# Yubo-Shankui/Bind-Your-Avatar-Implementation

Hardware: AMD Instinct MI355X
Metric: denoise-steps/sec (higher is better)
Workload: dtype bf16; 1 GPU; BASELINE.json configs[1]: full transformer.forward, 49x480x720 (13x30x45 latent tokens + 226 text), 2 characters (2 ID + 2 audio), batch 1, random-init 8.6B-param architecture; layers=42, batch=1, launch=eager, parallelism=single GPU

## Files before the change

### bind_your_avatar_implementation_amd/_hip.py

```python
import ctypes
import os

from .build import LIB_PATH as _BUILT_LIB

LIB_PATH = os.environ.get("BYA_HIP_LIB") or _BUILT_LIB

_c = ctypes
_vp, _i32, _i64, _f32 = _c.c_void_p, _c.c_int32, _c.c_int64, _c.c_float


class GemmDesc(_c.Structure):
    _fields_ = [("M", _i32), ("N", _i32), ("K", _i32), ("batch", _i32),
                ("lda", _i32), ("ldw", _i32), ("ldc", _i32), ("ldres", _i32),
                ("a_batch_stride", _i64), ("c_batch_stride", _i64), ("res_batch_stride", _i64),
                ("gate_batch_stride", _i64), ("gate_split", _i32), ("act", _i32),
                ("n_split", _i32), ("c_split_stride", _i64), ("bias_rowscale", _vp), ("alpha", _f32)]


class GemmPlan(_c.Structure):
    _fields_ = [("path", _i32), ("m0", _i32), ("tail", _i32), ("split_k", _i32), ("row_chunks", _i32)]


class QkNormDesc(_c.Structure):
    _fields_ = [("qw", _vp), ("qb", _vp), ("kw", _vp), ("kb", _vp), ("cos", _vp), ("sin", _vp),
# ... 165 lines not shown
                                 _i32, _i64, _i32, _vp],
    "bya_vae_conv3d": [_vp, _vp, _vp, _vp, _vp, _i32, _i32, _i32, _i32, _i32, _i32, _i64, _i64, _i64, _vp],
    "bya_vae_upsample_pad": [_vp, _vp, _i32, _i32, _i32, _i32, _i32, _vp],
    "bya_allgather_kv": [_vp, _vp, _vp, _vp, _i64, _i64, _vp, _vp],
    "bya_alltoall_router": [_vp, _vp, _vp, _vp, _i32, _vp, _vp],
    "bya_p2p_push": [_vp, _i32, _i64, _vp, _i32, _i32, _vp, _vp],
    "bya_p2p_wait": [_vp, _i32, _vp, _i64, _vp],
    "bya_p2p_exchange": [_vp, _i32, _i64, _vp, _i32, _i32, _vp, _vp, _i64, _vp],
    "bya_p2p_push_verified": [_vp, _i32, _i64, _vp, _i32, _i32, _vp, _vp, _vp, _vp, _vp, _vp],
    "bya_p2p_exchange_verified": [_vp, _i32, _i64, _vp, _i32, _i32, _vp, _vp, _i64, _vp, _vp, _vp, _vp, _vp],
    "bya_p2p_verify": [_vp, _vp, _vp, _i32, _i32, _vp, _vp, _vp],
    "bya_p2p_poison": [_vp, _i32, _vp, _i64, _vp],
    "bya_p2p_alloc": [_i64, _i32, _c.POINTER(_vp)],
    "bya_p2p_free": [_vp],
    "bya_p2p_ipc_export": [_vp, _vp],
    "bya_p2p_ipc_import": [_vp, _c.POINTER(_vp)],
    "bya_p2p_ipc_release": [_vp],
    "bya_cfg_scheduler_step": [_vp, _i32, _i64, _vp, _vp, _vp, _vp, _vp, _i64, _c.POINTER(SchedCoef), _vp],
    "bya_cfg_scheduler_step_plan": [_vp, _i32, _i64, _vp, _vp, _i64, _c.POINTER(SchedCoef), _c.POINTER(StepPlan)],
}

OPTIONS = {"gemm_splitk": 0, "gemm_splitk_min": 1, "gemm_tile": 2, "gemm_variant": 3, "attn_streamk": 4, "fp8_kernel": 5,
           "p2p_groups": 6, "reference_forms": 7, "mx_kernel": 8}
REFERENCE_FORMS = {"rowgemm_chunked": 1, "kv_mix_generic": 2, "ln_generic": 4, "router_scores_wave": 8, "attn_narrow_store": 16}
def _named_value(var, v, table):
    if v not in table:
        raise ValueError(f"{var}={v!r}: expected one of {sorted(table)}")
    return table[v]


ENV_OPTIONS = {
    "BYA_GEMM_SPLITK": ("gemm_splitk", int),
    "BYA_GEMM_SPLITK_MIN": ("gemm_splitk_min", int),
    "BYA_GEMM_TILE": ("gemm_tile", int),
    "BYA_GEMM_VARIANT": ("gemm_variant", lambda v: {"w8": 1, "no128": 2}.get(v, 0)),
    "BYA_ATTN_STREAMK": ("attn_streamk", int),
    "BYA_FP8_KERNEL": ("fp8_kernel", lambda v: 1 if v.startswith("1") else 0),
    "BYA_P2P_GROUPS": ("p2p_groups", int),
    "BYA_MX_KERNEL": ("mx_kernel", lambda v: _named_value("BYA_MX_KERNEL", v, {"0": 0, "1": 1, "p256": 1, "2": 2, "always": 2})),
}

GEMM_PATHS = {0: "t128x64", 1: "t128x128", 2: "t256x128", 3: "t256x256", 4: "p256", 5: "p128", 6: "p128s", 7: "w8_256"}

ATTN_VARIANTS = {0: "d64_running_max", 1: "d64_prescaled_running_max", 2: "d64_static_bound", 3: "d128_running_max",
                 4: "d64_static_bound_w4", 5: "d64_device_bound_w4"}
KV_MIX_FORMS = {0: "mix32", 1: "one_tile"}
TINY_INSTANCES = {0: "tiny8<2>", 1: "tiny8<3>", 2: "tiny8<13>", 3: "tiny8<25>", 4: "generic<2>", 5: "generic<4>",
# ... 61 lines not shown
```

### bind_your_avatar_implementation_amd/csrc/gemm_persistent.h

```cpp
#pragma once
#include "gemm_common.h"

namespace {

typedef int i32x4 __attribute__((ext_vector_type(4)));

struct XcdRange { int base, end; };
__host__ __device__ __forceinline__ XcdRange xcd_range(int total, int xcd) {
    const int cq = total >> 3, cr = total & 7;
    const int base = (xcd < cr) ? xcd * (cq + 1) : cr * (cq + 1) + (xcd - cr) * cq;
    return {base, base + cq + (xcd < cr ? 1 : 0)};
}

struct PersistentTile { int z, m0, n0; bool valid; };

template <int BM, int BN>
struct TileWalk {
    int tiles_m, tiles_n, per_z, gm;
    int base, end, slot, slots;
    __device__ __forceinline__ TileWalk(int tiles_m_, int tiles_n_, int batch, int gm_)
        : tiles_m(tiles_m_), tiles_n(tiles_n_), per_z(tiles_m_ * tiles_n_), gm(gm_) {
        const int total = per_z * batch, xcd = blockIdx.x & 7;
        slot = blockIdx.x >> 3;
        slots = gridDim.x >> 3;
// ... 34 lines not shown
__device__ __forceinline__ uint32_t stage_off96(int lane, int q, int rl, int src_row, uint32_t pitch) {
    const int b = (q * 1024 + lane * 16) % 96;
    return (uint32_t)src_row * pitch + (uint32_t)((b + 48 * ((rl >> 3) & 1)) % 96);
}

__device__ __forceinline__ i32x4 raw_rsrc(const void* base, uint32_t bytes) {
    const unsigned long long b = (unsigned long long)base;
    i32x4 r;
    r.x = __builtin_amdgcn_readfirstlane((int)(b & 0xffffffffu));
    r.y = __builtin_amdgcn_readfirstlane((int)((b >> 32) & 0xffffu));
    r.z = __builtin_amdgcn_readfirstlane((int)bytes);
    r.w = 0x00020000;
    return r;
}

template <int LDS_OFF = 0>
__device__ __forceinline__ void dma_piece(uint32_t lds_base, uint32_t voff, const i32x4& rsrc, uint32_t soff) {
    asm volatile("s_mov_b32 m0, %0\n\ts_nop 0\n\tbuffer_load_dwordx4 %1, %2, %3 offen lds"
                 :
                 : "s"(lds_base + LDS_OFF), "v"(voff), "s"(rsrc), "s"(soff)
                 : "memory");
}

template <typename T>
__device__ __forceinline__ i32x4 tile_rsrc_a(const GemmArgs& p, const T* A, const PersistentTile& c, int row_elems = 0) {
    const long long left = ((long long)(p.M - 1 - c.m0) * p.lda + (row_elems ? row_elems : p.K)) * (long long)sizeof(T);
    return raw_rsrc(A + (long long)c.z * p.a_bs + (long long)c.m0 * p.lda, c.valid && left > 0 ? (uint32_t)left : 0u);
}
template <typename T>
__device__ __forceinline__ i32x4 tile_rsrc_w(const GemmArgs& p, const T* W, const PersistentTile& c, int row_elems = 0) {
    const long long left = ((long long)(p.N - 1 - c.n0) * p.ldw + (row_elems ? row_elems : p.K)) * (long long)sizeof(T);
    return raw_rsrc(W + (long long)c.n0 * p.ldw, c.valid && left > 0 ? (uint32_t)left : 0u);
}

__device__ __forceinline__ uint32_t frag_addr(uint32_t tile, int row, int chunk) {
    return tile + row * 128 + ((chunk ^ ((row >> 1) & 7)) << 4);
}

__device__ __forceinline__ uint32_t frag_addr64(uint32_t tile, int row, int chunk) {
    return tile + row * 64 + ((chunk ^ (((row >> 2) & 1) << 1)) << 4);
}

__device__ __forceinline__ uint32_t frag_addr96(uint32_t tile, int row, int blk) {
    return tile + row * 96 + (blk ^ (((row >> 3) & 1) << 1)) * 24;
}

// ... 19 lines not shown
```

### bind_your_avatar_implementation_amd/csrc/gemm_v4.hip

```cpp
#include "gemm_wide_epilogue.h"
#include "options.h"

#ifndef BYA_GEMM_ABLATE
#define BYA_GEMM_ABLATE 0
#endif

namespace {

#ifdef BYA_GEMM_TIMELINE
#define TL_STAMP(K) do { if (!SPLIT && tid == 0 && p.ws_slabs) tl[K] = __builtin_amdgcn_s_memrealtime(); } while (0)
#else
#define TL_STAMP(K) do {} while (0)
#endif

struct TileCoord { int z, m0, n0; bool valid; int k0, nkk, role, parts, slab, slab_step, ctr; };
constexpr int DEFAULT_MIN_SPLIT_KTILES = 40;

template <bool SPLIT, bool CONV = false, bool QKN = false>
__global__ __launch_bounds__(256, 1) void gemm256p_kernel(GemmArgs p, int tiles_m, int tiles_n, int batch, int split_arg,
                                                          int min_seg, unsigned epoch) {
    static_assert(!(SPLIT && CONV), "the convolution instance does not split K");
    static_assert(!(QKN && (SPLIT || CONV)), "the q/k-norm instance is a plain, unsplit GEMM");
    const int split = SPLIT ? split_arg : 0;
    extern __shared__ __attribute__((aligned(16))) char smem[];
    constexpr int BM = 256, BN = 256, STAGE = (BM + BN) * BK * 2, TILE_A = BM * BK * 2;
    static_assert(STAGE == 65536, "stage flip uses one address bit");
    const int tid = threadIdx.x, lane = tid & 63;
    const int wave = __builtin_amdgcn_readfirstlane(tid >> 6);
    const int nk = p.K / BK;
    const int wm = wave >> 1, wn = wave & 1;
    const int fr = lane & 15, fq = lane >> 4;

    const int per_z = tiles_m * tiles_n, total = per_z * batch;
    const int xcd = blockIdx.x & 7, slot = blockIdx.x >> 3, slots = gridDim.x >> 3;
    const int cq = total >> 3, cr = total & 7;
    const int base = (xcd < cr) ? xcd * (cq + 1) : cr * (cq + 1) + (xcd - cr) * cq;
    const int end = base + cq + (xcd < cr ? 1 : 0);
    const int n_x = end - base;
    const int full = split ? n_x / slots : 0x7fffffff;
    const int R = split ? n_x - full * slots : 0;
    int parts = 1;
    if (split && R > 0) {
        parts = slots / R;
        if (parts > nk / min_seg) parts = nk / min_seg;
        if (parts < 1) parts = 1;
// ... 29 lines not shown
        constexpr int GM = BYA_GEMM_GM;
#else
        const int GM = p.gm;
#endif
        const int per_group = GM * tiles_n;
        const int group = idt / per_group, first_m = group * GM;
        const int gsz = (tiles_m - first_m) < GM ? (tiles_m - first_m) : GM;
        const int in_g = idt - group * per_group;
        c.m0 = (first_m + in_g % gsz) * BM;
        c.n0 = (in_g / gsz) * BN;
        return c;
    };
    int seq = 0;
    TileCoord cur = coord(seq);
    if (!cur.valid) return;

    const int a_row = wm * 128 + fr, w_row = wn * 128 + fr;
    const int a_sw = (a_row >> 1) & 7, w_sw = (w_row >> 1) & 7;
    const uint32_t lds0 = (uint32_t)(uintptr_t)LDS_PTR(smem);
    uint32_t cA0 = lds0 + a_row * 128 + ((fq ^ a_sw) << 4), cA1 = lds0 + a_row * 128 + (((4 + fq) ^ a_sw) << 4);
    uint32_t cW0 = lds0 + TILE_A + w_row * 128 + ((fq ^ w_sw) << 4);
    uint32_t cW1 = lds0 + TILE_A + w_row * 128 + (((4 + fq) ^ w_sw) << 4);
    uint32_t fill = __builtin_amdgcn_readfirstlane(lds0 + wave * 64 * 128);

    uint32_t voA[8], voW[8];
#pragma unroll
    for (int q = 0; q < 8; ++q) {
        const int rl = wave * 64 + q * 8 + (lane >> 3);
        const int wcol = w_slot_col(rl);
        const int chunk16 = ((lane & 7) ^ ((rl >> 1) & 7)) * 16;
        voA[q] = (uint32_t)rl * (uint32_t)(p.lda * 2) + chunk16;
        voW[q] = (uint32_t)wcol * (uint32_t)(p.ldw * 2) + chunk16;
    }
    auto a_rsrc = [&](const TileCoord& c) {
        long long left = CONV ? p.conv_a_bytes - (long long)c.m0 * p.lda * 2
                              : ((long long)(p.M - 1 - c.m0) * p.lda + p.K - c.k0 * BK) * 2;
        if (CONV && left > 0xffffffffLL) left = 0xffffffffLL;
        return raw_rsrc(p.A + (long long)c.z * p.a_bs + (long long)c.m0 * p.lda + c.k0 * BK,
                        c.valid && left > 0 ? (uint32_t)left : 0u);
    };
    auto w_rsrc = [&](const TileCoord& c) {
        const long long left = ((long long)(p.N - 1 - c.n0) * p.ldw + p.K - c.k0 * BK) * 2;
        return raw_rsrc(p.W + (long long)c.n0 * p.ldw + c.k0 * BK, c.valid && left > 0 ? (uint32_t)left : 0u);
    };
    i32x4 rsA = a_rsrc(cur), rsW = w_rsrc(cur);

// ... 5 lines not shown
    ALL8(DMA_W, fill ^ STAGE, voW, rsW, (uint32_t)(BK * 2));
    asm volatile("s_waitcnt vmcnt(16)" ::: "memory");

    f32x4 acc[8][8];
    bf16x8 fa[2][8], fw[2][8];

    for (;;) {
#ifdef BYA_GEMM_TIMELINE
        unsigned long long* const tl = reinterpret_cast<unsigned long long*>(p.ws_slabs + (size_t)(GEMM_WS_SLABS - 1) * (GEMM_WS_SLAB_BYTES / 4)) +
                                       ((size_t)blockIdx.x * 2 + (seq & 1)) * 8;
        TL_STAMP(0);
        if (!SPLIT && tid == 0 && p.ws_slabs) { tl[6] = (unsigned long long)cur.nkk; tl[7] = cur.valid ? 1ull : 0ull; }
#endif
        asm volatile("s_barrier" ::: "memory");
#define RA(S, J) ds_read128<(J) * 2048>(fa[S][J], (S) ? cA1 : cA0)
#define RW(S, I) ds_read128<(I) * 2048>(fw[S][I], (S) ? cW1 : cW0)
        RA(0, 0); RA(0, 1); RA(0, 2); RA(0, 3); RA(0, 4); RA(0, 5); RA(0, 6); RA(0, 7);
        RW(0, 0); RW(0, 1); RW(0, 2); RW(0, 3); RW(0, 4); RW(0, 5); RW(0, 6); RW(0, 7);
        asm volatile("s_waitcnt lgkmcnt(0)" ::: "memory");

        const TileCoord nxt = coord(seq + 1);
        const i32x4 rsAn = a_rsrc(nxt), rsWn = w_rsrc(nxt);
        const int unk = cur.nkk;

        auto ktile = [&](int t, auto v_c) {
            constexpr char V = decltype(v_c)::value;
            const uint32_t soff = (BYA_GEMM_ABLATE & 4) ? 0u : (uint32_t)((t + 2) * (BK * 2));
            uint32_t soffA = soff;
            if constexpr (CONV) {
                const uint32_t kt = (uint32_t)(t + 2), tap = kt >> p.conv_cpg_log2, cg = kt - (tap << p.conv_cpg_log2);
                const uint32_t dt = tap / 9u, r9 = tap - dt * 9u, dh = r9 / 3u, dw = r9 - dh * 3u;
                soffA = (((dt * (uint32_t)p.conv_Hp + dh) * (uint32_t)p.conv_Wp + dw) * (uint32_t)p.lda + cg * 64u) * 2u;
            }
#define MF(S, I, J) \
            asm volatile("v_mfma_f32_16x16x32_bf16 %0, %1, %2, %0" : "+a"(acc[I][J]) : "v"(fw[S][I]), "v"(fa[S][J]))
#define MFZ(S, I, J) \
            asm volatile("v_mfma_f32_16x16x32_bf16 %0, %1, %2, 0" : "=a"(acc[I][J]) : "v"(fw[S][I]), "v"(fa[S][J]))
#if BYA_GEMM_ABLATE & 1
#define DA(Q) do {} while (0)
#define DW(Q) do {} while (0)
#else
#define DA(Q) DMA_A(Q, fill, voA, rsA, soffA)
#define DW(Q) DMA_W(Q, fill, voW, rsW, soff)
#endif
#define PA(Q) DMA_A(Q, fill, voA, rsAn, 0u)
#define PW(Q) DMA_W(Q, fill, voW, rsWn, 0u)
#define QA(Q) DMA_A(Q, fill, voA, rsAn, (uint32_t)(BK * 2))
#define QW(Q) DMA_W(Q, fill, voW, rsWn, (uint32_t)(BK * 2))
#define WAIT_LGKM0() asm volatile("s_waitcnt lgkmcnt(0)" ::: "memory")
#define WAIT_VM(N) asm volatile("s_waitcnt vmcnt(" #N ")" ::: "memory")
#if BYA_GEMM_ABLATE & 2
#define BAR() do {} while (0)
#else
#define BAR() asm volatile("s_barrier" ::: "memory")
#endif
#define FLIP0() do { cA0 ^= STAGE; cW0 ^= STAGE; } while (0)
#define FLIP1() do { cA1 ^= STAGE; cW1 ^= STAGE; fill ^= STAGE; } while (0)
        if constexpr (V == 'A') {
            MFZ(0, 0, 0);  RA(1, 0);
            MFZ(0, 0, 1);  RA(1, 1);
            MFZ(0, 0, 2);  RA(1, 2);
            MFZ(0, 0, 3);  RA(1, 3);
            MFZ(0, 0, 4);  RA(1, 4);
            MFZ(0, 0, 5);  RA(1, 5);
            MFZ(0, 0, 6);  RA(1, 6);
            MFZ(0, 0, 7);  RA(1, 7);
            MFZ(0, 1, 0);
            MFZ(0, 1, 1);
            MFZ(0, 1, 2);
            MFZ(0, 1, 3);
            MFZ(0, 1, 4);
// ... 300 lines not shown
            MF(0, 6, 7);  WAIT_LGKM0();
            MF(0, 7, 0);
            MF(0, 7, 1);
            MF(0, 7, 2);
            MF(0, 7, 3);
            MF(0, 7, 4);
            MF(0, 7, 5);
            MF(0, 7, 6);
            MF(0, 7, 7);
            MF(1, 0, 0);
            MF(1, 0, 1);
            MF(1, 0, 2);
            MF(1, 0, 3);
            MF(1, 0, 4);
            MF(1, 0, 5);
            MF(1, 0, 6);
            MF(1, 0, 7);
            MF(1, 1, 0);
            MF(1, 1, 1);
            MF(1, 1, 2);
            MF(1, 1, 3);  WAIT_VM(0); BAR(); FLIP0();
            MF(1, 1, 4);  RA(0, 0);
            MF(1, 1, 5);  PA(0);
            MF(1, 1, 6);
            MF(1, 1, 7);  RA(0, 1);
            MF(1, 2, 0);  PA(1);
            MF(1, 2, 1);
            MF(1, 2, 2);  RA(0, 2);
            MF(1, 2, 3);  PA(2);
            MF(1, 2, 4);
            MF(1, 2, 5);  RA(0, 3);
            MF(1, 2, 6);  PA(3);
            MF(1, 2, 7);
            MF(1, 3, 0);  RA(0, 4);
            MF(1, 3, 1);  PA(4);
            MF(1, 3, 2);
            MF(1, 3, 3);  RA(0, 5);
            MF(1, 3, 4);  PA(5);
            MF(1, 3, 5);
            MF(1, 3, 6);  RA(0, 6);
            MF(1, 3, 7);  PA(6);
            MF(1, 4, 0);
            MF(1, 4, 1);  RA(0, 7);
            MF(1, 4, 2);  PA(7);
            MF(1, 4, 3);
            MF(1, 4, 4);  RW(0, 0);
            MF(1, 4, 5);  PW(0);
            MF(1, 4, 6);
            MF(1, 4, 7);  RW(0, 1);
            MF(1, 5, 0);  PW(1);
            MF(1, 5, 1);
            MF(1, 5, 2);  RW(0, 2);
            MF(1, 5, 3);  PW(2);
            MF(1, 5, 4);
            MF(1, 5, 5);  RW(0, 3);
            MF(1, 5, 6);  PW(3);
            MF(1, 5, 7);
            MF(1, 6, 0);  RW(0, 4);
            MF(1, 6, 1);  PW(4);
            MF(1, 6, 2);
            MF(1, 6, 3);  RW(0, 5);
            MF(1, 6, 4);  PW(5);
            MF(1, 6, 5);
            MF(1, 6, 6);  RW(0, 6);
            MF(1, 6, 7);  PW(6);
            MF(1, 7, 0);
            MF(1, 7, 1);  RW(0, 7);
            MF(1, 7, 2);  PW(7);
            MF(1, 7, 3);
            MF(1, 7, 4);
            MF(1, 7, 5);
// ... 118 lines not shown
            MF(1, 6, 3);
            MF(1, 6, 4);
            MF(1, 6, 5);
            MF(1, 6, 6);
            MF(1, 6, 7);
            MF(1, 7, 0);
            MF(1, 7, 1);
            MF(1, 7, 2);
            MF(1, 7, 3);
            MF(1, 7, 4);
            MF(1, 7, 5);
            MF(1, 7, 6);
            MF(1, 7, 7);  FLIP0(); FLIP1();
        }
            KEEP8(fa[0]); KEEP8(fw[0]); KEEP8(fa[1]); KEEP8(fw[1]);
#undef MF
#undef MFZ
#undef DA
#undef DW
#undef PA
#undef PW
#undef QA
#undef QW
#undef WAIT_LGKM0
#undef WAIT_VM
#undef BAR
#undef FLIP0
#undef FLIP1
        };
        ktile(0, IntTag<'A'>{});
        for (int t = 1; t + 2 < unk; ++t) ktile(t, IntTag<'B'>{});
        ktile(unk - 2, IntTag<'C'>{});
        ktile(unk - 1, IntTag<'D'>{});
#undef RA
#undef RW
        asm volatile("s_waitcnt vmcnt(16)\n\ts_nop 15\n\ts_nop 15" ::: "memory");
        TL_STAMP(1);

        if (SPLIT && cur.role == 2) {
            if (tid == 0) {
                int spins = 0;
                for (;;) {
                    const unsigned w = __hip_atomic_load(p.ws_counters + cur.ctr, __ATOMIC_RELAXED, __HIP_MEMORY_SCOPE_AGENT);
                    if ((w >> 8) == epoch && (w & 0xffu) >= (unsigned)(cur.parts - 1)) break;
                    __builtin_amdgcn_s_sleep(8);
                    if (++spins > (1 << 22)) {
                        __hip_atomic_fetch_add(p.ws_counters + 1023, 1u, __ATOMIC_RELAXED, __HIP_MEMORY_SCOPE_AGENT);
                        break;
                    }
                }
                if (split == 2) __builtin_amdgcn_fence(__ATOMIC_ACQUIRE, "agent");
            }
            asm volatile("s_waitcnt vmcnt(0)" ::: "memory");
            asm volatile("s_barrier" ::: "memory");
// ... 31 lines not shown
#pragma unroll
                            for (int i = 0; i < 8; ++i) ps[e][i] += c[e][i >> 2][i & 3];
                    }
#pragma unroll
                    for (int i = 0; i < 8; ++i) {
                        f32x4 t = acc[i][jn];
                        t[0] += ps[0][i]; t[1] += ps[1][i]; t[2] += ps[2][i]; t[3] += ps[3][i];
                        asm volatile("" : "+a"(t));
                        acc[i][jn] = t;
                    }
                }
            }
            auto run = [&](auto act_tag) {
                epilogue_wide<decltype(act_tag)::value, 2, SPLIT, CONV>(p, cur.z, cur.m0 + wm * 128, cur.n0 + wn * 128, fr, fq, acc, wave, lane);
            };
            dispatch_act_big(p.act, run);
            asm volatile("s_barrier" ::: "memory");
            if (tid == 0) __hip_atomic_store(p.ws_counters + cur.ctr, epoch << 8, __ATOMIC_RELAXED, __HIP_MEMORY_SCOPE_AGENT);
        } else {
            float* const raw_out = (SPLIT && cur.role == 1) ? p.ws_slabs + (size_t)cur.slab * (GEMM_WS_SLAB_BYTES / 4) : nullptr;
            if constexpr (QKN) {
                epilogue_qkn(p, cur.z, cur.m0 + wm * 128, cur.n0 + wn * 128, fr, fq, acc);
            } else {
                auto run = [&](auto act_tag) {
                    epilogue_wide<decltype(act_tag)::value, 2, SPLIT, CONV>(p, cur.z, cur.m0 + wm * 128, cur.n0 + wn * 128, fr, fq, acc,
                                                                            wave, lane, raw_out);
                };
                dispatch_act_big(p.act, run);
            }
            if (SPLIT && cur.role == 1) {
                asm volatile("s_waitcnt vmcnt(0)" ::: "memory");
                asm volatile("s_barrier" ::: "memory");
                if (tid == 0) {
                    if (split == 2) {
                        __builtin_amdgcn_fence(__ATOMIC_RELEASE, "agent");
                        asm volatile("s_waitcnt vmcnt(0)" ::: "memory");
                    }
                    unsigned* const c = p.ws_counters + cur.ctr;
                    unsigned old = __hip_atomic_load(c, __ATOMIC_RELAXED, __HIP_MEMORY_SCOPE_AGENT);
                    for (;;) {
                        const unsigned oe = old >> 8, age = (epoch - oe) & 0xffffffu;
                        unsigned want;
                        if (oe == epoch) want = old + 1u;
                        else if ((old & 0xffu) == 0u || age < 0x800000u) want = (epoch << 8) | 1u;
                        else break;
                        if (__hip_atomic_compare_exchange_strong(c, &old, want, __ATOMIC_RELAXED, __ATOMIC_RELAXED,
                                                                 __HIP_MEMORY_SCOPE_AGENT)) break;
                    }
                }
            }
        }
// ... 20 lines not shown
int bya_launch_gemm256p_qkn(const void* args, int batch, hipStream_t s) {
    GemmArgs a = *static_cast<const GemmArgs*>(args);
    a.gm = gemm_group_m(a);
    const int tiles_m = (a.M + 255) / 256, tiles_n = (a.N + 255) / 256;
    const size_t lds = 2 * 512 * BK * 2;
    return launch_persistent<gemm256p_kernel<false, false, true>>(persistent_grid((long long)tiles_m * tiles_n * batch), 256, lds, s, a, tiles_m, tiles_n,
                                                                  batch, 0, 1 << 30, 0u);
}

int bya_gemm_split_min_ktiles() {
    const int o = bya_opt(BYA_OPT_GEMM_SPLITK_MIN);
    const int v = o ? o : DEFAULT_MIN_SPLIT_KTILES;
    return v < 3 ? 3 : v;
}

int bya_gemm256p_split(const void* args, int batch) {
    const GemmArgs& a = *static_cast<const GemmArgs*>(args);
    const long long total = (long long)((a.M + 255) / 256) * ((a.N + 255) / 256) * batch;
    const int sk = bya_opt(BYA_OPT_GEMM_SPLITK);
    const int split = (a.ws_slabs && a.ws_counters && sk != 0 && a.K / BK >= 2 * bya_gemm_split_min_ktiles()) ? (sk == 2 ? 2 : 1) : 0;
    return total % 256 != 0 ? split : 0;
}

int bya_launch_gemm256p(const void* args, int batch, hipStream_t s) {
    GemmArgs a = *static_cast<const GemmArgs*>(args);
    a.gm = gemm_group_m(a);
    const int tiles_m = (a.M + 255) / 256, tiles_n = (a.N + 255) / 256;
    const long long total = (long long)tiles_m * tiles_n * batch;
    const int min_seg = bya_gemm_split_min_ktiles();
    const int split = bya_gemm256p_split(args, batch);
    const size_t lds = 2 * 512 * BK * 2;
    if (split) {
        static std::atomic<unsigned> g_epoch{0};
        unsigned epoch = (g_epoch.fetch_add(1) + 1u) & 0xffffffu;
        if (epoch == 0u) epoch = (g_epoch.fetch_add(1) + 1u) & 0xffffffu;
        return launch_persistent<gemm256p_kernel<true>>(256, 256, lds, s, a, tiles_m, tiles_n, batch, split, min_seg, epoch);
    }
    return launch_persistent<gemm256p_kernel<false>>(persistent_grid(total), 256, lds, s, a, tiles_m, tiles_n, batch, 0, min_seg, 0u);
}
```

### bind_your_avatar_implementation_amd/csrc/gemm_wide_epilogue.h

```cpp
#pragma once
#include "gemm_persistent.h"
#include "qknorm_math.h"
#include <type_traits>

namespace {

template <int ACT, int JB, bool SPLIT, bool CONV = false, int NJ = 8, bool PIN = false, bool SCALED = false>
__device__ __forceinline__ void epilogue_wide(const GemmArgs& p, int z, int m_wave, int n_wave, int fr, int fq,
                                              std::conditional_t<PIN, f32x4, const f32x4> (&acc)[8][NJ], int wave, int lane,
                                              float* raw_out = nullptr, const float* __restrict__ sa = nullptr,
                                              const float* __restrict__ sw = nullptr) {
    const bool has_res = p.res != nullptr, has_gate = p.gate0 != nullptr, has_bias = p.bias != nullptr;
    const bool has_rs = p.bias_rowscale != nullptr;
    const __amdgpu_buffer_rsrc_t rsR = __builtin_amdgcn_make_buffer_rsrc(
        (void*)((has_res ? p.res : p.C) + (long long)z * p.res_bs), 0, 0x7fffffff, 0x00020000);
    const __amdgpu_buffer_rsrc_t rsC = __builtin_amdgcn_make_buffer_rsrc(
        (void*)(p.C + (long long)z * p.c_bs), 0, 0x7fffffff, 0x00020000);
    const char* g0base = reinterpret_cast<const char*>(p.gate0 + (long long)z * p.gate_bs);
    const char* g1base = reinterpret_cast<const char*>(p.gate1 + (long long)z * p.gate_bs);
    u32x4 bv[4], g0[4], g1[4];
    f32x4 wv[4][2];
    uint32_t ncb[4], colb[4];
    bool nok[4];
#pragma unroll
    for (int e = 0; e < 4; ++e) {
        const int n8 = n_wave + (4 * e + fq) * 8;
        nok[e] = n8 < p.N;
        ncb[e] = nok[e] ? (uint32_t)n8 * 2u : 0u;
        colb[e] = (uint32_t)n8 * 2u;
        if (p.n_split > 0) colb[e] = ((uint32_t)(n8 / p.n_split) * (uint32_t)p.c_split_stride + (uint32_t)(n8 % p.n_split)) * 2u;
        bv[e] = has_bias ? *reinterpret_cast<const u32x4*>(reinterpret_cast<const char*>(p.bias) + ncb[e]) : u32x4{0u, 0u, 0u, 0u};
        if constexpr (SCALED) {
            wv[e][0] = *reinterpret_cast<const f32x4*>(sw + (nok[e] ? n8 : 0));
            wv[e][1] = *reinterpret_cast<const f32x4*>(sw + (nok[e] ? n8 : 0) + 4);
        }
        if (has_gate) {
            g0[e] = *reinterpret_cast<const u32x4*>(g0base + ncb[e]);
            g1[e] = *reinterpret_cast<const u32x4*>(g1base + ncb[e]);
        }
    }
#pragma unroll
    for (int jb = 0; jb < NJ; jb += JB) {
        u32x4 rv[JB][4];
        float rs[JB], ra[JB];
        bool mok[JB];
        uint32_t roff[JB], coff[JB];
        if constexpr (PIN) {
#pragma unroll
            for (int jj = 0; jj < JB; ++jj)
#pragma unroll
                for (int i = 0; i < 8; ++i) asm volatile("" : "+a"(acc[i][jb + jj]));
        }
#pragma unroll
        for (int jj = 0; jj < JB; ++jj) {
            const int m = m_wave + 16 * (jb + jj) + fr;
            mok[jj] = m < p.M;
            uint32_t mc = mok[jj] ? (uint32_t)m : 0u;
            if constexpr (CONV) {
                const uint32_t plane = (uint32_t)(p.conv_Hp * p.conv_Wp);
                const uint32_t t = mc / plane, rem = mc - t * plane;
                const uint32_t h = rem / (uint32_t)p.conv_Wp, w = rem - h * (uint32_t)p.conv_Wp;
                mok[jj] = mok[jj] && h < (uint32_t)p.conv_H && w < (uint32_t)p.conv_W && t < (uint32_t)p.conv_To;
                mc = mok[jj] ? (t * (uint32_t)p.conv_H + h) * (uint32_t)p.conv_W + w : 0u;
            }
            rs[jj] = has_rs ? p.bias_rowscale[(long long)z * p.M + mc] : 1.0f;
            if constexpr (SCALED) ra[jj] = sa[(long long)z * p.M + mc];
            roff[jj] = mc * (uint32_t)(p.ldres * 2);
            coff[jj] = mc * (uint32_t)(p.ldc * 2);
            if (has_res) {
#pragma unroll
                for (int e = 0; e < 4; ++e)
                    rv[jj][e] = __builtin_bit_cast(u32x4, __builtin_amdgcn_raw_buffer_load_b128(
                        rsR, (mok[jj] && nok[e]) ? roff[jj] + ncb[e] : 0xffffffffu, 0, 0));
            }
        }
#pragma unroll
        for (int jj = 0; jj < JB; ++jj) {
            const int j = jb + jj;
            const int m = m_wave + 16 * j + fr;
#pragma unroll
            for (int e = 0; e < 4; ++e) {
                float b8[8], v[8], a0[8];
#pragma unroll
                for (int i = 0; i < 8; ++i) {
                    if constexpr (SCALED) a0[i] = acc[i][j][e] * (ra[jj] * wv[e][i >> 2][i & 3]);
                    else a0[i] = acc[i][j][e];
                }
                if (SPLIT && raw_out) {
                    const __amdgpu_buffer_rsrc_t rsS = __builtin_amdgcn_make_buffer_rsrc((void*)raw_out, 0, (int)GEMM_WS_SLAB_BYTES, 0x00020000);
                    const uint32_t so = (uint32_t)(((wave * 64 + (j * 4 + e) * 2) * 64 + lane) * 16);
                    float one = 1.0f;
                    asm volatile("" : "+s"(one));
                    const f32x4 lof = {a0[0] * one, a0[1] * one, a0[2] * one, a0[3] * one};
                    const f32x4 hif = {a0[4] * one, a0[5] * one, a0[6] * one, a0[7] * one};
                    const u32x4 lo = __builtin_bit_cast(u32x4, lof), hi = __builtin_bit_cast(u32x4, hif);
                    __builtin_amdgcn_raw_buffer_store_b128(lo, rsS, so, 0, 16 );
                    __builtin_amdgcn_raw_buffer_store_b128(hi, rsS, so + 1024, 0, 16 );
                    continue;
                }
                unpack8(bv[e], b8);
#pragma unroll
                for (int i = 0; i < 8; ++i) v[i] = p.alpha * apply_act<ACT>(fmaf(rs[jj], b8[i], a0[i]), p.leaky);
                if (has_gate) {
                    float g8[8];
                    unpack8(m < p.gate_split ? g0[e] : g1[e], g8);
#pragma unroll
                    for (int i = 0; i < 8; ++i) v[i] *= g8[i];
                }
                if (has_res) {
                    float r8[8];
                    unpack8(rv[jj][e], r8);
#pragma unroll
                    for (int i = 0; i < 8; ++i) v[i] += r8[i];
                }
                __builtin_amdgcn_raw_buffer_store_b128(pack8(v), rsC, (mok[jj] && nok[e]) ? coff[jj] + colb[e] : 0xffffffffu, 0, 0);
            }
        }
    }
}

template <int NJ = 8>
__device__ __forceinline__ void epilogue_qkn(const GemmArgs& p, int z, int m_wave, int n_wave, int fr, int fq, const f32x4 (&acc)[8][NJ]) {
    const __amdgpu_buffer_rsrc_t rsC = __builtin_amdgcn_make_buffer_rsrc((void*)(p.C + (long long)z * p.c_bs), 0, 0x7fffffff, 0x00020000);
    const int tsel = n_wave / p.qkn_width;
    const bool has_bias = p.bias != nullptr;
    u32x4 bv[4];
    uint32_t colb[4];
    bool nok[4];
// ... 171 lines not shown
```

### bind_your_avatar_implementation_amd/csrc/misc.hip

```cpp
#include "bya_common.h"
#include "../../include/bya.h"
#include "options.h"
#include "routing_weights.h"

namespace {

template <int MAXM>
__global__ __launch_bounds__(256) void linear_small_m_kernel(const bf16_t* __restrict__ x, const bf16_t* __restrict__ W,
                                                             const bf16_t* __restrict__ bias, bf16_t* __restrict__ out,
                                                             int M, int N, int K, int silu_in, int act_out) {
    const int lane = threadIdx.x & 63;
    const long long n = (long long)blockIdx.x * 4 + (threadIdx.x >> 6);
    if (n >= N) return;
    float acc[MAXM];
#pragma unroll
    for (int m = 0; m < MAXM; ++m) acc[m] = 0.f;
    const bf16_t* wrow = W + n * K;
    for (int k0 = lane * 8; k0 < K; k0 += 512) {
        float wv[8];
        unpack8(*reinterpret_cast<const u32x4*>(wrow + k0), wv);
#pragma unroll
        for (int m = 0; m < MAXM; ++m) {
            if (m < M) {
                float xv[8];
// ... 274 lines not shown
        if (v > 0.5f) label = id;
    }
    for (int id = 0; id < n_id; ++id) out[tok * n_id + id] = (id == label) ? (bf16_t)0x3F80 : (bf16_t)0;
}

}

extern "C" int bya_abi_version(void) { return 2; }

std::atomic<int32_t> g_bya_options[BYA_OPT_COUNT] = {
    {0},
    {0},
    {-1},
    {0},
    {1},
    {0},
    {0},
    {0},
    {0},
};

extern "C" int bya_set_option(int32_t key, int32_t value) {
    static const int32_t lo[BYA_OPT_COUNT] = {0, 0, -1, 0, 0, 0, 0, 0, 0};
    static const int32_t hi[BYA_OPT_COUNT] = {2, 1 << 20, 6, 2, 1, 1, 1024, 31, 2};
    if (key < 0 || key >= BYA_OPT_COUNT || value < lo[key] || value > hi[key]) return BYA_ERR_SHAPE;
    if (key == BYA_OPT_P2P_GROUPS && value != 0 && value < 16) return BYA_ERR_SHAPE;
    g_bya_options[key].store(value, std::memory_order_relaxed);
    return BYA_OK;
}

extern "C" int bya_get_option(int32_t key, int32_t* value) {
    if (key < 0 || key >= BYA_OPT_COUNT || !value) return BYA_ERR_SHAPE;
    *value = g_bya_options[key].load(std::memory_order_relaxed);
    return BYA_OK;
}

static int small_m_plan_of(const void* x, const void* W, const void* out, int32_t M, int32_t N, int32_t K, int32_t act_out,
                           bya_step_plan_info* p) {
    if (!x || !W || !out || M <= 0 || M > 8 || N <= 0 || K <= 0) return BYA_ERR_SHAPE;
    if (K % 8) return BYA_ERR_SHAPE;
    if (((uintptr_t)x | (uintptr_t)W) & 15) return BYA_ERR_ALIGN;
    if (act_out != BYA_ACT_NONE && act_out != BYA_ACT_SILU) return BYA_ERR_UNSUPPORTED;
    p->kernel = M <= 2 ? 2 : 8;
    p->grid = (N + 3) / 4;
    p->rounds = (K + 511) / 512;
    p->reserved = 0;
    p->items = N;
// ... 182 lines not shown
```

### include/bya.h

```cpp
#ifndef BYA_H
#define BYA_H

#include <stdint.h>

#ifdef __cplusplus
extern "C" {
#endif
#if defined(__GNUC__) || defined(__clang__)
#pragma GCC visibility push(default)
#endif

#ifndef __HIP_PLATFORM_AMD__
typedef struct ihipStream_t* hipStream_t;
#endif

enum { BYA_ACT_NONE = 0, BYA_ACT_GELU_TANH = 1, BYA_ACT_GELU_ERF = 2, BYA_ACT_RELU = 3, BYA_ACT_SILU = 4,
       BYA_ACT_LEAKY_RELU = 5,
       BYA_ACT_GELU_TANH_IEEE = 6  };

int bya_abi_version(void);

enum bya_option {
    BYA_OPT_GEMM_SPLITK = 0,
    BYA_OPT_GEMM_SPLITK_MIN = 1,
    BYA_OPT_GEMM_TILE = 2,
    BYA_OPT_GEMM_VARIANT = 3,
    BYA_OPT_ATTN_STREAMK = 4,
    BYA_OPT_FP8_KERNEL = 5,
    BYA_OPT_P2P_GROUPS = 6,
    BYA_OPT_REFERENCE_FORMS = 7,
    BYA_OPT_MX_KERNEL = 8,
    BYA_OPT_COUNT = 9
};
enum { BYA_REF_ROWGEMM_CHUNKED = 1,
       BYA_REF_KV_MIX_GENERIC = 2,
       BYA_REF_LN_GENERIC = 4,
       BYA_REF_ROUTER_SCORES_WAVE = 8,
       BYA_REF_ATTN_NARROW_STORE = 16   };
int bya_set_option(int32_t key, int32_t value);
int bya_get_option(int32_t key, int32_t* value);

#define BYA_CALIBRATION_OPERAND_BYTES (256LL * 256 * 16 * 16)
#define BYA_CALIBRATION_FLOP_PER_ITER (256.0 * 4 * 2.0 * 128 * 128 * 32)
int bya_mfma_calibration(const void* operands, int64_t operand_bytes, void* sink, int32_t iters, hipStream_t stream);

typedef struct bya_gemm_desc {
    int32_t M, N, K;
    int32_t batch;
    int32_t lda, ldw, ldc, ldres;
    int64_t a_batch_stride, c_batch_stride, res_batch_stride, gate_batch_stride;
    int32_t gate_split;
    int32_t act;
    int32_t n_split;
    int64_t c_split_stride;
    const float* bias_rowscale;
    float alpha;
} bya_gemm_desc;

int bya_gemm_bf16(const void* A, const void* W, const void* bias, void* C, const void* res,
                  const void* gate0, const void* gate1, const bya_gemm_desc* desc, hipStream_t stream);

// ... 420 lines not shown
```

Before: 2.784 steps/s.

## Prefetch GEMM epilogue operands into LDS during the last K-tiles

For the persistent 256x256 GEMM with a residual and no activation, bias, gate, residual first-row-block and row-scale operands are DMA'd into a per-wave LDS staging area, with the loads interleaved into the MFMA schedule of the final K-tiles. The remaining residual rows are requested early in the epilogue. This hides epilogue global-load latency behind matrix math instead of stalling after the main loop. It costs extra LDS per block and adds complexity to the hand-scheduled pipeline; an option can disable it.

```diff
diff --git a/bind_your_avatar_implementation_amd/_hip.py b/bind_your_avatar_implementation_amd/_hip.py
--- a/bind_your_avatar_implementation_amd/_hip.py
+++ b/bind_your_avatar_implementation_amd/_hip.py
@@ -211,7 +211,8 @@
 
 OPTIONS = {"gemm_splitk": 0, "gemm_splitk_min": 1, "gemm_tile": 2, "gemm_variant": 3, "attn_streamk": 4, "fp8_kernel": 5,
            "p2p_groups": 6, "reference_forms": 7, "mx_kernel": 8}
-REFERENCE_FORMS = {"rowgemm_chunked": 1, "kv_mix_generic": 2, "ln_generic": 4, "router_scores_wave": 8, "attn_narrow_store": 16}
+REFERENCE_FORMS = {"rowgemm_chunked": 1, "kv_mix_generic": 2, "ln_generic": 4, "router_scores_wave": 8, "attn_narrow_store": 16,
+                   "gemm_epilogue_unstaged": 32}
 def _named_value(var, v, table):
     if v not in table:
         raise ValueError(f"{var}={v!r}: expected one of {sorted(table)}")
diff --git a/bind_your_avatar_implementation_amd/csrc/gemm_persistent.h b/bind_your_avatar_implementation_amd/csrc/gemm_persistent.h
--- a/bind_your_avatar_implementation_amd/csrc/gemm_persistent.h
+++ b/bind_your_avatar_implementation_amd/csrc/gemm_persistent.h
@@ -80,6 +80,14 @@
                  : "memory");
 }
 
+template <int LDS_OFF = 0>
+__device__ __forceinline__ void dma_piece4(uint32_t lds_base, uint32_t voff, const i32x4& rsrc, uint32_t soff) {
+    asm volatile("s_mov_b32 m0, %0\n\ts_nop 0\n\tbuffer_load_dword %1, %2, %3 offen lds"
+                 :
+                 : "s"(lds_base + LDS_OFF), "v"(voff), "s"(rsrc), "s"(soff)
+                 : "memory");
+}
+
 template <typename T>
 __device__ __forceinline__ i32x4 tile_rsrc_a(const GemmArgs& p, const T* A, const PersistentTile& c, int row_elems = 0) {
     const long long left = ((long long)(p.M - 1 - c.m0) * p.lda + (row_elems ? row_elems : p.K)) * (long long)sizeof(T);
diff --git a/bind_your_avatar_implementation_amd/csrc/gemm_v4.hip b/bind_your_avatar_implementation_amd/csrc/gemm_v4.hip
--- a/bind_your_avatar_implementation_amd/csrc/gemm_v4.hip
+++ b/bind_your_avatar_implementation_amd/csrc/gemm_v4.hip
@@ -9,18 +9,23 @@
 
 #ifdef BYA_GEMM_TIMELINE
 #define TL_STAMP(K) do { if (!SPLIT && tid == 0 && p.ws_slabs) tl[K] = __builtin_amdgcn_s_memrealtime(); } while (0)
+#define TL_ARG , (!SPLIT && p.ws_slabs) ? tl : nullptr
 #else
 #define TL_STAMP(K) do {} while (0)
+#define TL_ARG
 #endif
+
+__device__ __forceinline__ int fresh_lane() { return (int)__builtin_amdgcn_mbcnt_hi(~0u, __builtin_amdgcn_mbcnt_lo(~0u, 0u)); }
 
 struct TileCoord { int z, m0, n0; bool valid; int k0, nkk, role, parts, slab, slab_step, ctr; };
 constexpr int DEFAULT_MIN_SPLIT_KTILES = 40;
 
-template <bool SPLIT, bool CONV = false, bool QKN = false>
+template <bool SPLIT, bool CONV = false, bool QKN = false, bool EPI_STAGE = false>
 __global__ __launch_bounds__(256, 1) void gemm256p_kernel(GemmArgs p, int tiles_m, int tiles_n, int batch, int split_arg,
                                                           int min_seg, unsigned epoch) {
     static_assert(!(SPLIT && CONV), "the convolution instance does not split K");
     static_assert(!(QKN && (SPLIT || CONV)), "the q/k-norm instance is a plain, unsplit GEMM");
+    static_assert(!(EPI_STAGE && (SPLIT || CONV || QKN)), "epilogue operands are staged for the plain, unsplit GEMM only");
     const int split = SPLIT ? split_arg : 0;
     extern __shared__ __attribute__((aligned(16))) char smem[];
     constexpr int BM = 256, BN = 256, STAGE = (BM + BN) * BK * 2, TILE_A = BM * BK * 2;
@@ -96,6 +101,7 @@
     uint32_t cW0 = lds0 + TILE_A + w_row * 128 + ((fq ^ w_sw) << 4);
     uint32_t cW1 = lds0 + TILE_A + w_row * 128 + (((4 + fq) ^ w_sw) << 4);
     uint32_t fill = __builtin_amdgcn_readfirstlane(lds0 + wave * 64 * 128);
+    const uint32_t stg = __builtin_amdgcn_readfirstlane(lds0 + 2 * STAGE + wave * GEMM_EPI_STAGE_WAVE_BYTES);
 
     uint32_t voA[8], voW[8];
 #pragma unroll
@@ -147,6 +153,9 @@
         const TileCoord nxt = coord(seq + 1);
         const i32x4 rsAn = a_rsrc(nxt), rsWn = w_rsrc(nxt);
         const int unk = cur.nkk;
+        i32x4 rsSB = {0, 0, 0, 0}, rsSG0 = {0, 0, 0, 0}, rsSG1 = {0, 0, 0, 0}, rsSR = {0, 0, 0, 0}, rsSS = {0, 0, 0, 0};
+        uint32_t svr = 0u;
+        int svn = 0, sn_wave = 0, sm_wave = 0;
 
         auto ktile = [&](int t, auto v_c) {
             constexpr char V = decltype(v_c)::value;
@@ -172,6 +181,19 @@
 #define PW(Q) DMA_W(Q, fill, voW, rsWn, 0u)
 #define QA(Q) DMA_A(Q, fill, voA, rsAn, (uint32_t)(BK * 2))
 #define QW(Q) DMA_W(Q, fill, voW, rsWn, (uint32_t)(BK * 2))
+#define SE(Q) do { if constexpr (EPI_STAGE) { \
+                if constexpr ((Q) < 3) { \
+                    const int nv = sn_wave + (fresh_lane() & 15) * 8;             \
+                    const uint32_t svv = nv < p.N ? (uint32_t)nv * 2u : 0xffffffffu; \
+                    if constexpr ((Q) == 0) dma_piece<0>(stg, svv, rsSB, 0u); \
+                    else if constexpr ((Q) == 1) dma_piece<1024>(stg, svv, rsSG0, 0u); \
+                    else dma_piece<2048>(stg, svv, rsSG1, 0u); \
+                } else if constexpr ((Q) < 7) { \
+                    dma_piece<(Q) * 1024>(stg, 32 * ((Q) - 3) < svn ? svr + 64u * ((Q) - 3) : 0xffffffffu, rsSR, 0u); \
+                } else {                                                          \
+                    const int ms = sm_wave + 64 * ((Q) - 7) + fresh_lane(); \
+                    dma_piece4<GEMM_EPI_STAGE_ROWSCALE + ((Q) - 7) * 256>(stg, ms < p.M ? (uint32_t)ms * 4u : 0xffffffffu, rsSS, 0u); \
+                } } } while (0)
 #define WAIT_LGKM0() asm volatile("s_waitcnt lgkmcnt(0)" ::: "memory")
 #define WAIT_VM(N) asm volatile("s_waitcnt vmcnt(" #N ")" ::: "memory")
 #if BYA_GEMM_ABLATE & 2
@@ -518,31 +540,31 @@
             MF(1, 1, 3);  WAIT_VM(0); BAR(); FLIP0();
             MF(1, 1, 4);  RA(0, 0);
             MF(1, 1, 5);  PA(0);
-            MF(1, 1, 6);
+            MF(1, 1, 6);  SE(0);
             MF(1, 1, 7);  RA(0, 1);
             MF(1, 2, 0);  PA(1);
-            MF(1, 2, 1);
+            MF(1, 2, 1);  SE(1);
             MF(1, 2, 2);  RA(0, 2);
             MF(1, 2, 3);  PA(2);
-            MF(1, 2, 4);
+            MF(1, 2, 4);  SE(2);
             MF(1, 2, 5);  RA(0, 3);
             MF(1, 2, 6);  PA(3);
-            MF(1, 2, 7);
+            MF(1, 2, 7);  SE(3);
             MF(1, 3, 0);  RA(0, 4);
             MF(1, 3, 1);  PA(4);
-            MF(1, 3, 2);
+            MF(1, 3, 2);  SE(4);
             MF(1, 3, 3);  RA(0, 5);
             MF(1, 3, 4);  PA(5);
-            MF(1, 3, 5);
+            MF(1, 3, 5);  SE(5);
             MF(1, 3, 6);  RA(0, 6);
             MF(1, 3, 7);  PA(6);
-            MF(1, 4, 0);
+            MF(1, 4, 0);  SE(6);
             MF(1, 4, 1);  RA(0, 7);
             MF(1, 4, 2);  PA(7);
-            MF(1, 4, 3);
+            MF(1, 4, 3);  SE(7);
             MF(1, 4, 4);  RW(0, 0);
             MF(1, 4, 5);  PW(0);
-            MF(1, 4, 6);
+            MF(1, 4, 6);  SE(8);
             MF(1, 4, 7);  RW(0, 1);
             MF(1, 5, 0);  PW(1);
             MF(1, 5, 1);
@@ -707,6 +729,7 @@
 #undef PW
 #undef QA
 #undef QW
+#undef SE
 #undef WAIT_LGKM0
 #undef WAIT_VM
 #undef BAR
@@ -715,6 +738,23 @@
         };
         ktile(0, IntTag<'A'>{});
         for (int t = 1; t + 2 < unk; ++t) ktile(t, IntTag<'B'>{});
+        if constexpr (EPI_STAGE) {
+            const int ln = fresh_lane(), fr = ln & 15, fq = ln >> 4;
+            sn_wave = cur.n0 + wn * 128;
+            sm_wave = cur.m0 + wm * 128;
+            const int m = sm_wave + fr;
+            svr = (uint32_t)m * (uint32_t)(p.ldres * 2) + (uint32_t)(sn_wave + fq * 8) * 2u;
+            svn = m < p.M ? p.N - sn_wave - fq * 8 : 0;
+            auto rsrc = [](const void* base, bool present) {
+                const unsigned long long b = (unsigned long long)base;
+                return i32x4{(int)(b & 0xffffffffu), (int)((b >> 32) & 0xffffu), present ? 0x7fffffff : 0, 0x00020000};
+            };
+            rsSB = rsrc(p.bias, p.bias != nullptr);
+            rsSG0 = rsrc(p.gate0 + (long long)cur.z * p.gate_bs, p.gate0 != nullptr);
+            rsSG1 = rsrc(p.gate1 + (long long)cur.z * p.gate_bs, p.gate0 != nullptr);
+            rsSR = rsrc(p.res + (long long)cur.z * p.res_bs, p.res != nullptr);
+            rsSS = rsrc(p.bias_rowscale + (long long)cur.z * p.M, p.bias_rowscale != nullptr);
+        }
         ktile(unk - 2, IntTag<'C'>{});
         ktile(unk - 1, IntTag<'D'>{});
 #undef RA
@@ -792,11 +832,16 @@
             if constexpr (QKN) {
                 epilogue_qkn(p, cur.z, cur.m0 + wm * 128, cur.n0 + wn * 128, fr, fq, acc);
             } else {
+                const int ln = EPI_STAGE ? fresh_lane() : lane, fre = EPI_STAGE ? (ln & 15) : fr, fqe = EPI_STAGE ? (ln >> 4) : fq;
                 auto run = [&](auto act_tag) {
-                    epilogue_wide<decltype(act_tag)::value, 2, SPLIT, CONV>(p, cur.z, cur.m0 + wm * 128, cur.n0 + wn * 128, fr, fq, acc,
-                                                                            wave, lane, raw_out);
+                    epilogue_wide<decltype(act_tag)::value, 2, SPLIT, CONV, 8, false, false, EPI_STAGE>(
+                        p, cur.z, cur.m0 + wm * 128, cur.n0 + wn * 128, fre, fqe, acc, wave, ln, raw_out, nullptr, nullptr, stg TL_ARG);
                 };
-                dispatch_act_big(p.act, run);
+                if constexpr (EPI_STAGE) {
+                    run(IntTag<0>{});
+                } else {
+                    dispatch_act_big(p.act, run);
+                }
             }
             if (SPLIT && cur.role == 1) {
                 asm volatile("s_waitcnt vmcnt(0)" ::: "memory");
@@ -863,6 +908,14 @@
     return total % 256 != 0 ? split : 0;
 }
 
+#ifndef BYA_GEMM_EPI_STAGE_MAX_KTILES
+#define BYA_GEMM_EPI_STAGE_MAX_KTILES 96
+#endif
+bool bya_gemm256p_stages_epilogue(const void* args) {
+    const GemmArgs& a = *static_cast<const GemmArgs*>(args);
+    return a.res && a.act == 0 && a.K / BK <= BYA_GEMM_EPI_STAGE_MAX_KTILES && !bya_ref_form(BYA_REF_GEMM_EPILOGUE_UNSTAGED);
+}
+
 int bya_launch_gemm256p(const void* args, int batch, hipStream_t s) {
     GemmArgs a = *static_cast<const GemmArgs*>(args);
     a.gm = gemm_group_m(a);
@@ -877,5 +930,8 @@
         if (epoch == 0u) epoch = (g_epoch.fetch_add(1) + 1u) & 0xffffffu;
         return launch_persistent<gemm256p_kernel<true>>(256, 256, lds, s, a, tiles_m, tiles_n, batch, split, min_seg, epoch);
     }
+    if (bya_gemm256p_stages_epilogue(&a))
+        return launch_persistent<gemm256p_kernel<false, false, false, true>>(persistent_grid(total), 256, lds + 4 * GEMM_EPI_STAGE_WAVE_BYTES, s, a,
+                                                                             tiles_m, tiles_n, batch, 0, min_seg, 0u);
     return launch_persistent<gemm256p_kernel<false>>(persistent_grid(total), 256, lds, s, a, tiles_m, tiles_n, batch, 0, min_seg, 0u);
 }
diff --git a/bind_your_avatar_implementation_amd/csrc/gemm_wide_epilogue.h b/bind_your_avatar_implementation_amd/csrc/gemm_wide_epilogue.h
--- a/bind_your_avatar_implementation_amd/csrc/gemm_wide_epilogue.h
+++ b/bind_your_avatar_implementation_amd/csrc/gemm_wide_epilogue.h
@@ -5,11 +5,27 @@
 
 namespace {
 
-template <int ACT, int JB, bool SPLIT, bool CONV = false, int NJ = 8, bool PIN = false, bool SCALED = false>
+constexpr int GEMM_EPI_STAGE_BIAS = 0, GEMM_EPI_STAGE_GATE0 = 1024, GEMM_EPI_STAGE_GATE1 = 2048, GEMM_EPI_STAGE_RES = 3072;
+constexpr int GEMM_EPI_STAGE_ROWSCALE = 7168;
+constexpr int GEMM_EPI_STAGE_WAVE_BYTES = 7680;
+
+__device__ __forceinline__ uint32_t lds_load32(uint32_t addr) {
+    return *(const __attribute__((address_space(3))) uint32_t*)(uintptr_t)addr;
+}
+__device__ __forceinline__ u32x4 lds_load128(uint32_t addr) {
+    return *(const __attribute__((address_space(3))) u32x4*)(uintptr_t)addr;
+}
+
+template <int ACT, int JB, bool SPLIT, bool CONV = false, int NJ = 8, bool PIN = false, bool SCALED = false, bool STAGED = false>
 __device__ __forceinline__ void epilogue_wide(const GemmArgs& p, int z, int m_wave, int n_wave, int fr, int fq,
                                               std::conditional_t<PIN, f32x4, const f32x4> (&acc)[8][NJ], int wave, int lane,
                                               float* raw_out = nullptr, const float* __restrict__ sa = nullptr,
-                                              const float* __restrict__ sw = nullptr) {
+                                              const float* __restrict__ sw = nullptr, uint32_t stg = 0u
+#ifdef BYA_GEMM_TIMELINE
+                                              , unsigned long long* tl = nullptr
+#endif
+                                              ) {
+    static_assert(!(STAGED && (SPLIT || CONV || PIN || SCALED)), "operands are staged for the plain bf16 epilogue only");
     const bool has_res = p.res != nullptr, has_gate = p.gate0 != nullptr, has_bias = p.bias != nullptr;
     const bool has_rs = p.bias_rowscale != nullptr;
     const __amdgpu_buffer_rsrc_t rsR = __builtin_amdgcn_make_buffer_rsrc(
@@ -29,6 +45,9 @@
         ncb[e] = nok[e] ? (uint32_t)n8 * 2u : 0u;
         colb[e] = (uint32_t)n8 * 2u;
         if (p.n_split > 0) colb[e] = ((uint32_t)(n8 / p.n_split) * (uint32_t)p.c_split_stride + (uint32_t)(n8 % p.n_split)) * 2u;
+        if constexpr (STAGED) {
+            continue;
+        }
         bv[e] = has_bias ? *reinterpret_cast<const u32x4*>(reinterpret_cast<const char*>(p.bias) + ncb[e]) : u32x4{0u, 0u, 0u, 0u};
         if constexpr (SCALED) {
             wv[e][0] = *reinterpret_cast<const f32x4*>(sw + (nok[e] ? n8 : 0));
@@ -38,6 +57,24 @@
             g0[e] = *reinterpret_cast<const u32x4*>(g0base + ncb[e]);
             g1[e] = *reinterpret_cast<const u32x4*>(g1base + ncb[e]);
         }
+    }
+    u32x4 rvs[STAGED ? NJ : 1][4];
+    const __amdgpu_buffer_rsrc_t rsRq = __builtin_amdgcn_make_buffer_rsrc(
+        (void*)((has_res ? p.res : p.C) + (long long)z * p.res_bs), 0, has_res ? 0x7fffffff : 0, 0x00020000);
+    auto request_res = [&](int j) {
+        const int m = m_wave + 16 * j + fr;
+        const uint32_t ro = (uint32_t)m * (uint32_t)(p.ldres * 2);
+#pragma unroll
+        for (int e = 0; e < 4; ++e)
+            rvs[STAGED ? j : 0][e] = __builtin_bit_cast(u32x4, __builtin_amdgcn_raw_buffer_load_b128(
+                rsRq, ((m < p.M) & nok[e]) ? ro + ncb[e] : 0xffffffffu, 0, 0));
+    };
+    if constexpr (STAGED) {
+#pragma unroll
+        for (int j = 1; j < NJ; ++j) request_res(j);
+        __builtin_amdgcn_sched_barrier(0);
+#pragma unroll
+        for (int e = 0; e < 4; ++e) rvs[0][e] = lds_load128(stg + GEMM_EPI_STAGE_RES + e * 1024 + lane * 16);
     }
 #pragma unroll
     for (int jb = 0; jb < NJ; jb += JB) {
@@ -63,17 +100,27 @@
                 mok[jj] = mok[jj] && h < (uint32_t)p.conv_H && w < (uint32_t)p.conv_W && t < (uint32_t)p.conv_To;
                 mc = mok[jj] ? (t * (uint32_t)p.conv_H + h) * (uint32_t)p.conv_W + w : 0u;
             }
-            rs[jj] = has_rs ? p.bias_rowscale[(long long)z * p.M + mc] : 1.0f;
+            if constexpr (STAGED) rs[jj] = has_rs ? __builtin_bit_cast(float, lds_load32(stg + GEMM_EPI_STAGE_ROWSCALE + (16 * (jb + jj) + fr) * 4)) : 1.0f;
+            else rs[jj] = has_rs ? p.bias_rowscale[(long long)z * p.M + mc] : 1.0f;
             if constexpr (SCALED) ra[jj] = sa[(long long)z * p.M + mc];
             roff[jj] = mc * (uint32_t)(p.ldres * 2);
             coff[jj] = mc * (uint32_t)(p.ldc * 2);
             if (has_res) {
 #pragma unroll
-                for (int e = 0; e < 4; ++e)
-                    rv[jj][e] = __builtin_bit_cast(u32x4, __builtin_amdgcn_raw_buffer_load_b128(
+                for (int e = 0; e < 4; ++e) {
+                    if constexpr (STAGED) rv[jj][e] = rvs[jb + jj][e];
+                    else rv[jj][e] = __builtin_bit_cast(u32x4, __builtin_amdgcn_raw_buffer_load_b128(
                         rsR, (mok[jj] && nok[e]) ? roff[jj] + ncb[e] : 0xffffffffu, 0, 0));
-            }
-        }
+                }
+            }
+        }
+#ifdef BYA_GEMM_TIMELINE
+        if (jb == 0 && tl) {
+            if constexpr (STAGED) asm volatile("s_waitcnt lgkmcnt(0)" ::: "memory");
+            else asm volatile("s_waitcnt vmcnt(0) lgkmcnt(0)" ::: "memory");
+            if (threadIdx.x == 0) tl[2] = __builtin_amdgcn_s_memrealtime();
+        }
+#endif
 #pragma unroll
         for (int jj = 0; jj < JB; ++jj) {
             const int j = jb + jj;
@@ -98,12 +145,15 @@
                     __builtin_amdgcn_raw_buffer_store_b128(hi, rsS, so + 1024, 0, 16 );
                     continue;
                 }
-                unpack8(bv[e], b8);
+                const uint32_t cv = stg + (uint32_t)((4 * e + fq) * 16);
+                if constexpr (STAGED) unpack8(lds_load128(cv + GEMM_EPI_STAGE_BIAS), b8);
+                else unpack8(bv[e], b8);
 #pragma unroll
                 for (int i = 0; i < 8; ++i) v[i] = p.alpha * apply_act<ACT>(fmaf(rs[jj], b8[i], a0[i]), p.leaky);
                 if (has_gate) {
                     float g8[8];
-                    unpack8(m < p.gate_split ? g0[e] : g1[e], g8);
+                    if constexpr (STAGED) unpack8(lds_load128(cv + (m < p.gate_split ? GEMM_EPI_STAGE_GATE0 : GEMM_EPI_STAGE_GATE1)), g8);
+                    else unpack8(m < p.gate_split ? g0[e] : g1[e], g8);
 #pragma unroll
                     for (int i = 0; i < 8; ++i) v[i] *= g8[i];
                 }
diff --git a/bind_your_avatar_implementation_amd/csrc/misc.hip b/bind_your_avatar_implementation_amd/csrc/misc.hip
--- a/bind_your_avatar_implementation_amd/csrc/misc.hip
+++ b/bind_your_avatar_implementation_amd/csrc/misc.hip
@@ -320,7 +320,7 @@
 
 extern "C" int bya_set_option(int32_t key, int32_t value) {
     static const int32_t lo[BYA_OPT_COUNT] = {0, 0, -1, 0, 0, 0, 0, 0, 0};
-    static const int32_t hi[BYA_OPT_COUNT] = {2, 1 << 20, 6, 2, 1, 1, 1024, 31, 2};
+    static const int32_t hi[BYA_OPT_COUNT] = {2, 1 << 20, 6, 2, 1, 1, 1024, 63, 2};
     if (key < 0 || key >= BYA_OPT_COUNT || value < lo[key] || value > hi[key]) return BYA_ERR_SHAPE;
     if (key == BYA_OPT_P2P_GROUPS && value != 0 && value < 16) return BYA_ERR_SHAPE;
     g_bya_options[key].store(value, std::memory_order_relaxed);
diff --git a/include/bya.h b/include/bya.h
--- a/include/bya.h
+++ b/include/bya.h
@@ -36,7 +36,8 @@
        BYA_REF_KV_MIX_GENERIC = 2,
        BYA_REF_LN_GENERIC = 4,
        BYA_REF_ROUTER_SCORES_WAVE = 8,
-       BYA_REF_ATTN_NARROW_STORE = 16   };
+       BYA_REF_ATTN_NARROW_STORE = 16,
+       BYA_REF_GEMM_EPILOGUE_UNSTAGED = 32  };
 int bya_set_option(int32_t key, int32_t value);
 int bya_get_option(int32_t key, int32_t* value);
 
```

Result: no change. 2.780 steps/s (-0.1%).
